# willow-ahrens/ChainPartitioners.jl

Measured on AMD Instinct MI355X. Metric: partitions/sec, DynamicTotalSplitter(AffineConnectivityModel{Int64}(0,0,0,1)), K=64, higher is better.
Workload: dtype int64; 1 GPU; config 3: DynamicTotalSplitter(AffineConnectivityModel{Int64}(0,0,0,1)) on suitesparse_shaped CSR (seeded SplitMix64 generator, tests/synth.py), n=10000000 rows, nnz=100000000, K=64; one independent partition per GPU; n=10000000, nnz=100000000, K=64, includes_oracle_build=True, device_block_pool=True

## Files before the change

### chainpartitioners.jl_amd/csrc/dp_total.hip

```cpp
#include "csr.hpp"
#include "model.hpp"
#include "dp.hpp"
#include <algorithm>

namespace cpk {

template <typename TC>
__device__ __forceinline__ TC dm_apply_affine(const DevModel<TC> &m, TC alpha, int64_t nv, int64_t np, int64_t nn, int64_t nl)
{
    TC v = cadd(cadd(alpha, cmulc(nv, m.p[CP_P_VERTEX])), cmulc(np, m.p[CP_P_PIN]));
    if (m.kind == CP_MODEL_CONNECTIVITY) return cadd(v, cmulc(nn, m.p[CP_P_NET]));
    if (m.kind == CP_MODEL_HYPEREDGE_CUT) return cadd(cadd(v, cmulc(nl, m.p[CP_P_SELF_NET])), cmulc(nn - nl, m.p[CP_P_CUT_NET]));
    return v;
}
#define dm_apply dm_apply_affine

constexpr int LT = 256;
constexpr int NBMAX = 31;
constexpr int SPLIT_BMIN = 8;
constexpr int SPLIT_NB = NBMAX - SPLIT_BMIN;

__device__ __forceinline__ int64_t prow(int64_t r, int64_t n)
{
    int t = __ffsll((long long)r) - 1;
// ... 558 lines not shown
    }
}

__device__ __forceinline__ void load_tile_tasks(const int64_t *__restrict__ offs, int64_t ntask, int64_t t0, int64_t tile_start,
                                                bool active, int32_t *s_off, unsigned long long *s_hd, int lane, int &cnt)
{
    int64_t c = ntask - t0;
    cnt = active ? (int)(c > LT + 1 ? LT + 1 : c) : 0;
    if (lane < LT / 64) s_hd[lane] = 0ull;
    for (int i = lane; i < cnt; i += 64) {
        int64_t rel = offs[t0 + i] - tile_start;
        if (rel < -(int64_t)0x3fffffff) rel = -(int64_t)0x3fffffff;
        if (rel > (int64_t)0x3fffffff) rel = (int64_t)0x3fffffff;
        s_off[i] = (int32_t)rel;
        if (rel >= 0 && rel < LT) atomicOr(&s_hd[rel >> 6], 1ull << (rel & 63));
    }
}

template <bool GE>
__device__ __forceinline__ int32_t coop_count(const int32_t *__restrict__ arr, int32_t s, int32_t en, int32_t thr, bool valid, int lane)
{
    int32_t prev_s = __shfl_up(s, 1);
    int prev_valid = __shfl_up((int)valid, 1);
    bool cont = valid && lane > 0 && prev_valid && (en == prev_s);
    unsigned long long heads = __ballot(valid && !cont);
    unsigned long long vm = __ballot(valid);
    int32_t d = 0;
    const int32_t FILL = GE ? INT32_MIN : INT32_MAX;
    while (heads) {
        int h0 = __ffsll((long long)heads) - 1;
        heads &= heads - 1;
        int h1 = heads ? (__ffsll((long long)heads) - 1) : 64;
        unsigned long long inrun = vm & (h1 == 64 ? ~0ull : ((1ull << h1) - 1)) & ~((1ull << h0) - 1);
        int hl = 63 - __clzll((long long)inrun);
        int32_t q_hi = __shfl(en, h0), q_lo = __shfl(s, hl);
        bool mine = lane >= h0 && lane <= hl && en > s;
        for (int32_t x = q_lo & ~3; x < q_hi; x += 512) {
            int4 v0 = make_int4(FILL, FILL, FILL, FILL), v1 = v0;
            int32_t b0 = x + 4 * lane, b1 = b0 + 256;
            if (b0 < q_hi) v0 = *reinterpret_cast<const int4 *>(arr + b0);
            if (b1 < q_hi) v1 = *reinterpret_cast<const int4 *>(arr + b1);
#pragma unroll
            for (int c = 0; c < 2; c++) {
                int32_t xc = x + c * 256;
                if (xc >= q_hi) break;
                int4 v = c ? v1 : v0;
                bool ov = mine && s < xc + 256 && en > xc;
                int a0 = ov ? ((s > xc ? s : xc) - xc) : 0, a1 = ov ? ((en < xc + 256 ? en : xc + 256) - xc) : 0;
                unsigned long long rem = __ballot(ov);
                while (rem) {
                    int l = __ffsll((long long)rem) - 1;
                    int32_t tu = __shfl(thr, l);
                    const bool f0 = GE ? v.x >= tu : v.x < tu, f1 = GE ? v.y >= tu : v.y < tu, f2 = GE ? v.z >= tu : v.z < tu, f3 = GE ? v.w >= tu : v.w < tu;
                    const unsigned long long m0 = __ballot(f0), m1 = __ballot(f1), m2 = __ballot(f2), m3 = __ballot(f3);
                    uint32_t P0 = 0;
                    P0 = __builtin_amdgcn_mbcnt_hi((uint32_t)(m0 >> 32), __builtin_amdgcn_mbcnt_lo((uint32_t)m0, P0));
                    P0 = __builtin_amdgcn_mbcnt_hi((uint32_t)(m1 >> 32), __builtin_amdgcn_mbcnt_lo((uint32_t)m1, P0));
                    P0 = __builtin_amdgcn_mbcnt_hi((uint32_t)(m2 >> 32), __builtin_amdgcn_mbcnt_lo((uint32_t)m2, P0));
                    P0 = __builtin_amdgcn_mbcnt_hi((uint32_t)(m3 >> 32), __builtin_amdgcn_mbcnt_lo((uint32_t)m3, P0));
                    const int32_t pack = (int32_t)((P0 << 3) | (uint32_t)f0 | ((uint32_t)f1 << 1) | ((uint32_t)f2 << 2));
                    const int32_t tot = __popcll(m0) + __popcll(m1) + __popcll(m2) + __popcll(m3);
                    const int32_t g0 = __shfl(pack, (a0 >> 2) & 63), g1 = __shfl(pack, (a1 >> 2) & 63);
                    bool same = ov && thr == tu;
                    if (same) {
                        int32_t F0 = (g0 >> 3) + __popc((uint32_t)g0 & ((1u << (a0 & 3)) - 1u));
                        int32_t F1 = a1 >= 256 ? tot : (g1 >> 3) + __popc((uint32_t)g1 & ((1u << (a1 & 3)) - 1u));
                        d += F1 - F0;
                    }
                    rem &= ~__ballot(same);
                }
            }
        }
    }
    return d;
}

constexpr int SMAX = 31;
template <bool GE, bool DET = false>
__device__ __forceinline__ void interior_stream(const int32_t *__restrict__ arr, const int32_t *__restrict__ cpos, int32_t p_first, int32_t tl,
                                                int32_t thr, int lane, int32_t acc[4], int32_t sk[4], int head = 0, int32_t sp_lo = 0, int32_t sp_hi = 0,
                                                int32_t *s_es = nullptr, int32_t *s_v = nullptr, int32_t *s_cnt = nullptr, int kind = 0,
                                                const int32_t *__restrict__ psum = nullptr)
{
    const int32_t FILL = GE ? INT32_MIN : INT32_MAX;
    const int32_t ptop = psum ? psum[p_first + 1 - head] : 0;
#pragma unroll
    for (int k = 0; k < 4; k++) {
        int32_t e = lane + 64 * k;
        sk[k] = e <= tl ? cpos[p_first - e] : INT32_MAX;
        acc[k] = (psum && e <= tl) ? ptop - psum[p_first - e] : 0;
    }
    int32_t Q_hi = cpos[p_first + 1 - head], Q_lo = cpos[p_first - tl];
    int32_t x = Q_lo & ~3;
    int4 c0 = make_int4(FILL, FILL, FILL, FILL), c1 = c0;
    if (x + 4 * lane < Q_hi) c0 = *reinterpret_cast<const int4 *>(arr + x + 4 * lane);
    if (x + 256 + 4 * lane < Q_hi) c1 = *reinterpret_cast<const int4 *>(arr + x + 256 + 4 * lane);
    for (; x < Q_hi; x += 512) {
        int4 n0 = make_int4(FILL, FILL, FILL, FILL), n1 = n0;
        if (x + 512 + 4 * lane < Q_hi) n0 = *reinterpret_cast<const int4 *>(arr + x + 512 + 4 * lane);
        if (x + 768 + 4 * lane < Q_hi) n1 = *reinterpret_cast<const int4 *>(arr + x + 768 + 4 * lane);
#pragma unroll
        for (int c = 0; c < 2; c++) {
            int32_t xc = x + c * 256;
            if (xc >= Q_hi) break;
            int4 v = c ? c1 : c0;
            int32_t pb = xc + 4 * lane;
            const bool inner = xc >= Q_lo && xc + 256 <= Q_hi;
            bool f0 = GE ? v.x >= thr : v.x < thr, f1 = GE ? v.y >= thr : v.y < thr, f2 = GE ? v.z >= thr : v.z < thr, f3 = GE ? v.w >= thr : v.w < thr;
            if (!inner) { f0 = f0 && pb < Q_hi; f1 = f1 && pb + 1 < Q_hi; f2 = f2 && pb + 2 < Q_hi; f3 = f3 && pb + 3 < Q_hi; }
            const unsigned long long m0 = __ballot(f0), m1 = __ballot(f1), m2 = __ballot(f2), m3 = __ballot(f3);
            if (DET) {
                const uint32_t span = (uint32_t)(sp_hi - sp_lo - 1);
                bool s0 = (uint32_t)(v.x - sp_lo - 1) < span, s1 = (uint32_t)(v.y - sp_lo - 1) < span, s2 = (uint32_t)(v.z - sp_lo - 1) < span,
                     s3 = (uint32_t)(v.w - sp_lo - 1) < span;
                if (!inner) {
                    s0 = s0 && pb >= Q_lo && pb < Q_hi; s1 = s1 && pb + 1 >= Q_lo && pb + 1 < Q_hi;
                    s2 = s2 && pb + 2 >= Q_lo && pb + 2 < Q_hi; s3 = s3 && pb + 3 >= Q_lo && pb + 3 < Q_hi;
                }
                if (s0 || s1 || s2 || s3) {
#pragma unroll
                    for (int j = 0; j < 4; j++) {
                        if (j == 0 ? s0 : j == 1 ? s1 : j == 2 ? s2 : s3) {
                            int32_t val = j == 0 ? v.x : j == 1 ? v.y : j == 2 ? v.z : v.w;
                            int slot = atomicAdd(s_cnt, 1);
                            if (slot <= SMAX - 1) {
                                s_es[slot] = pb + j;
                                s_v[slot] = (int32_t)(((uint32_t)val & 0x7fffffffu) | ((uint32_t)kind << 31));
                            }
                        }
                    }
                }
            }
            int32_t tot = __popcll(m0) + __popcll(m1) + __popcll(m2) + __popcll(m3);
            uint32_t P0 = 0;
            P0 = __builtin_amdgcn_mbcnt_hi((uint32_t)(m0 >> 32), __builtin_amdgcn_mbcnt_lo((uint32_t)m0, P0));
            P0 = __builtin_amdgcn_mbcnt_hi((uint32_t)(m1 >> 32), __builtin_amdgcn_mbcnt_lo((uint32_t)m1, P0));
            P0 = __builtin_amdgcn_mbcnt_hi((uint32_t)(m2 >> 32), __builtin_amdgcn_mbcnt_lo((uint32_t)m2, P0));
            P0 = __builtin_amdgcn_mbcnt_hi((uint32_t)(m3 >> 32), __builtin_amdgcn_mbcnt_lo((uint32_t)m3, P0));
            const int32_t pack = (int32_t)((P0 << 3) | (uint32_t)f0 | ((uint32_t)f1 << 1) | ((uint32_t)f2 << 2));
#pragma unroll
            for (int k = 0; k < 4; k++) {
                int32_t idx = sk[k] - xc;
                bool inside = idx > 0 && idx < 256;
                if (__ballot(inside)) {
                    int32_t cidx = inside ? idx : 0;
                    int src = cidx >> 2, comp = cidx & 3;
                    const int32_t g = __shfl(pack, src);
                    int32_t Fb = (g >> 3) + __popc((uint32_t)g & ((1u << comp) - 1u));
                    acc[k] += idx <= 0 ? tot : (inside ? tot - Fb : 0);
                } else {
                    acc[k] += idx <= 0 ? tot : 0;
                }
            }
        }
        c0 = n0; c1 = n1;
    }
}

constexpr int FIX_SERIAL = 16;
constexpr int FIX_U = 8;
constexpr int FIX_TRIP = 256 * FIX_U;
__global__ void __launch_bounds__(256) k_own_map(RoundCounts *__restrict__ rc, const int64_t *__restrict__ toffs, const int4 *__restrict__ tdesc,
                                                 const int32_t *__restrict__ rlen, int4 *__restrict__ rec, int32_t *__restrict__ tile_task,
                                                 const uint8_t *__restrict__ tb, int32_t *__restrict__ gap_hi, int tau, int64_t n, int blk,
                                                 int32_t *__restrict__ bcnt, int32_t *__restrict__ brank, int2 *__restrict__ items,
                                                 int32_t *__restrict__ item_of, int split)
{
    const int64_t ntask = rc->nown, ntile = rc->NT;
    for (int64_t tile = (int64_t)blockIdx.x * blockDim.x + threadIdx.x; tile < ntile; tile += (int64_t)gridDim.x * blockDim.x) {
    int64_t lo = 0, hi = ntask;
    while (hi - lo > 1) {
        int64_t mid = (lo + hi) >> 1;
        if (toffs[mid] <= tile) lo = mid; else hi = mid;
    }
    int32_t kt = (int32_t)(tile - toffs[lo]);
    if (items) {
        const bool first = kt % FIX_TRIP == 0 && toffs[lo + 1] - toffs[lo] > FIX_SERIAL;
        const unsigned long long mf = __ballot(first);
        if (mf) {
            const int lane = threadIdx.x & 63, lead = __ffsll((long long)mf) - 1;
            int32_t base = 0;
            if (lane == lead) base = atomicAdd(&rc->n_items, (int32_t)__popcll(mf));
            base = __shfl(base, lead);
            if (first) {
                const int32_t it = base + __popcll(mf & ((1ull << lane) - 1ull));
                items[it] = make_int2((int32_t)lo, kt);
                item_of[tile] = it;
            }
        }
    }
    int4 td = tdesc[lo];
    int32_t pf, tl;
    own_tile_geo(blk, td.x, rlen[lo], kt, pf, tl);
    const bool isgap = gap_hi != nullptr;
    const int sb = (split && tb[lo] >= SPLIT_BMIN) ? tb[lo] : 0;
    rec[tile] = make_int4(pf, td.z, td.w, (sb << 10) | (tl << 2) | (isgap ? 2 : 0) | (kt == 0 ? 1 : 0));
    if (split == 2) {
        const unsigned long long ms = __ballot(sb != 0);
        if (ms && (int)(threadIdx.x & 63) == __ffsll((long long)ms) - 1) atomicAdd(&rc->n_split, (int32_t)__popcll(ms));
    }
    tile_task[tile] = (int32_t)lo;
    if (bcnt) brank[tile] = atomicAdd(&bcnt[pf / LT], 1);
    if (isgap) {
        int64_t r = td.z, b = tb[lo];
        int64_t hi = r + ((int64_t)1 << tau), re = (((r >> b) + 1) << b);
        if (hi > re) hi = re;
        if (hi > n + 1) hi = n + 1;
        gap_hi[tile] = (int32_t)hi;
    }
    }
}

__global__ void __launch_bounds__(256) k_blk_order(const RoundCounts *__restrict__ rc, const int4 *__restrict__ rec, const int32_t *__restrict__ brank,
                                                   const int64_t *__restrict__ bstart, int32_t *__restrict__ border, int32_t *__restrict__ bcnt)
{
    const int64_t ntile = rc->NT;
    for (int64_t tile = (int64_t)blockIdx.x * blockDim.x + threadIdx.x; tile < ntile; tile += (int64_t)gridDim.x * blockDim.x) {
        const int32_t c = rec[tile].x / LT, rk = brank[tile];
        border[bstart[c] + rk] = (int32_t)tile;
        if (rk == 0) bcnt[c] = 0;
    }
}

template <typename TC, bool HYP, bool GAP>
__global__ void __launch_bounds__(256) k_lpass_own(int isA, const RoundCounts *__restrict__ rc, const int32_t *__restrict__ border,
                                                   const int32_t *__restrict__ a_pos, const int32_t *__restrict__ a_next,
                                                   const int32_t *__restrict__ a_fpos, const int32_t *__restrict__ a_flast,
                                                   int32_t *__restrict__ a_tileS, int32_t *__restrict__ a_tileS2, const int4 *__restrict__ a_rec,
                                                   const TC *__restrict__ W, DevModel<TC> M, TC alpha, Best<TC, HYP> *__restrict__ part,
                                                   int tau, const int32_t *__restrict__ gap_hi, uint8_t *__restrict__ spec, int force_spec,
                                                   Best<TC, HYP> *__restrict__ sub, int32_t *__restrict__ spv,
                                                   const int32_t *__restrict__ a_col, const int32_t *__restrict__ a_ffirst,
                                                   const int32_t *__restrict__ a_vnext, const int32_t *__restrict__ a_vpos,
                                                   const int32_t *__restrict__ a_vsa, int64_t vstride)
{
    int lane = threadIdx.x & 63;
    int64_t tile = (int64_t)blockIdx.x * 4 + (threadIdx.x >> 6);
    if (tile >= rc->NT) return;
    if (border) tile = border[tile];
    int4 rec = a_rec[tile];
    const int32_t rw = __builtin_amdgcn_readfirstlane(rec.w);
    int head = rw & 1;
    int32_t tl = (rw >> 2) & 255;
    int32_t acc[4], acc2[4] = {0, 0, 0, 0}, sk[4], sk2[4];
    __shared__ int32_t s_es_all[4][2][SMAX + 1], s_v_all[4][2][SMAX + 1];
    __shared__ int32_t s_cnt_all[4];
    int32_t(*s_es)[SMAX + 1] = s_es_all[threadIdx.x >> 6], (*s_v)[SMAX + 1] = s_v_all[threadIdx.x >> 6];
    int ns = 0;
    if (GAP && (rw & 2)) {
        int32_t *s_cnt = &s_cnt_all[threadIdx.x >> 6];
        if (lane == 0) *s_cnt = 0;
        __threadfence_block();
        int32_t rL = rec.y - (1 << tau), hi1 = gap_hi[tile] - 1;
        interior_stream<true, true>(a_next, a_pos, rec.x, tl, hi1, lane, acc, sk, head, rL, hi1, s_es[0], s_v[0], s_cnt, 0);
        if (HYP) interior_stream<false, true>(a_flast, a_fpos, rec.x, tl, rL + 1, lane, acc2, sk2, head, rL, hi1, s_es[0], s_v[0], s_cnt, 1);
        __threadfence_block();
        ns = *s_cnt;
        if (force_spec) ns = SMAX + 1;
        if (ns > 0 && ns <= SMAX) {
            if (lane < ns) {
                const int32_t q = s_es[0][lane];
                const bool k1 = s_v[0][lane] < 0;
                s_es[0][lane] = rec.x - (k1 ? a_ffirst[q] : a_col[q]);
            }
            __threadfence_block();
        }
    } else if (!HYP && !GAP) {
        const int sb = rw >> 10;
        const int64_t so = sb ? (int64_t)(sb - SPLIT_BMIN) * vstride : 0;
        interior_stream<true>(sb ? a_vnext : a_next, sb ? a_vpos + so : a_pos, rec.x, tl, rec.y, lane, acc, sk, head, 0, 0, nullptr, nullptr, nullptr, 0,
                              sb ? a_vsa + so : (const int32_t *)nullptr);
        if (sb) {
#pragma unroll
            for (int k = 0; k < 4; k++) if (lane + 64 * k <= tl) sk[k] = a_pos[rec.x - lane - 64 * k];
        }
    } else {
        interior_stream<true>(a_next, a_pos, rec.x, tl, rec.y, lane, acc, sk, head);
        if (HYP) interior_stream<false>(a_flast, a_fpos, rec.x, tl, rec.y, lane, acc2, sk2, head);
    }
    int sel = tl >> 6;
    if (lane == (tl & 63)) {
        a_tileS[tile] = sel == 0 ? acc[0] : sel == 1 ? acc[1] : sel == 2 ? acc[2] : acc[3];
        if (HYP) a_tileS2[tile] = sel == 0 ? acc2[0] : sel == 1 ? acc2[1] : sel == 2 ? acc2[2] : acc2[3];
    }
    Best<TC, HYP> cand[4];
#pragma unroll
    for (int k = 0; k < 4; k++) {
        int32_t e = lane + 64 * k;
        best_clear(cand[k]);
        if (e <= tl && !(head && isA && e == 0)) {
            int32_t p = rec.x - e;
            TC fv = dm_apply(M, alpha, (int64_t)(rec.y - p), (int64_t)(rec.z - sk[k]), (int64_t)acc[k], (int64_t)acc2[k]);
            cand[k].v = cadd(W[p], fv); cand[k].p = p; cand[k].nn = acc[k]; best_set_nl(cand[k], acc2[k]);
        }
    }
    if (GAP && ns > SMAX) {
        if (lane == 0) spec[tile] = 255;
        return;
    }
    if (!GAP || ns == 0) {
        Best<TC, HYP> best; best_clear(best);
#pragma unroll
        for (int k = 0; k < 4; k++) best = better(best, cand[k]);
        for (int o = 32; o > 0; o >>= 1) {
            int src = (lane + o) & 63;
            Best<TC, HYP> c; best_clear(c); c.v = shfl64(best.v, src); c.p = __shfl(best.p, src); c.nn = __shfl(best.nn, src);
            if (HYP) best_set_nl(c, __shfl(best_nl(best), src));
            bool take = (best.p < 0) ? (c.p >= 0) : (c.p >= 0 && (c.v < best.v || (c.v == best.v && c.p > best.p)));
            if (lane + o < 64 && take) best = c;
        }
        if (lane == 0) { part[tile] = best; if (GAP) spec[tile] = 0; }
        return;
    }
    __threadfence_block();
    if (lane < ns) {
        int32_t es_i = s_es[0][lane]; int rank = 0;
        for (int j = 0; j < ns; j++) { int32_t es_j = s_es[0][j]; rank += (es_j < es_i) || (es_j == es_i && j < lane); }
        s_es[1][rank] = es_i; s_v[1][rank] = s_v[0][lane];
    }
    __threadfence_block();
    int seg[4] = {0, 0, 0, 0}, hd[5] = {0, 0, 0, 0, 0};
    for (int i = 0; i < ns; i++) {
        int32_t es_i = s_es[1][i];
#pragma unroll
        for (int k = 0; k < 4; k++) { seg[k] += (es_i <= lane + 64 * k); hd[k] |= (es_i == lane + 64 * k); }
    }
    if (lane == 0) hd[0] = 1;
    const int64_t sbase = tile * (SMAX + 1);
    if (lane <= ns) {
        int32_t lo = lane == 0 ? 0 : s_es[1][lane - 1], hi = lane == ns ? tl + 1 : s_es[1][lane];
        if (hi <= lo) { Best<TC, HYP> z; best_clear(z); sub[sbase + lane] = z; }
    }
    Best<TC, HYP> bcarry; best_clear(bcarry);
#pragma unroll
    for (int k = 0; k < 4; k++) {
        int32_t e = lane + 64 * k;
        Best<TC, HYP> x = cand[k];
        int f = hd[k];
        wave_segmin<TC, HYP>(x, f, lane);
        if (!f) x = better(bcarry, x);
        {
            Best<TC, HYP> nb; best_clear(nb); nb.v = shfl64(x.v, 63); nb.p = __shfl(x.p, 63); nb.nn = __shfl(x.nn, 63);
            if (HYP) best_set_nl(nb, __shfl(best_nl(x), 63));
            bcarry = nb;
        }
        int nh = __shfl_down(hd[k], 1), nh0 = __shfl(hd[k + 1], 0);
        if (lane == 63) nh = nh0;
        if (e <= tl && (e == tl || nh)) sub[sbase + seg[k]] = x;
    }
    if (lane < ns) spv[sbase + lane] = s_v[1][lane];
    if (lane == 0) spec[tile] = (uint8_t)ns;
}

template <bool GE>
__device__ __forceinline__ int32_t gap_right_counts(const int32_t *__restrict__ cpos, const int32_t *__restrict__ arr, int32_t rL, int ck, int32_t thr,
                                                    int32_t n, int lane)
{
    int32_t cfirst = rL + 64 * ck;
    if (cfirst > n) cfirst = n;
    int32_t c = 0;
    for (int32_t q = cpos[rL] + lane, q1 = cpos[cfirst]; q < q1; q += 64) { int32_t v = arr[q]; c += GE ? (v >= thr) : (v < thr); }
    for (int o = 32; o > 0; o >>= 1) c += __shfl_xor(c, o);
    int32_t jn = cfirst + lane + 1, cl = cfirst + 64;
    if (jn > n) jn = n;
    if (cl > n) cl = n;
    const int32_t myend = cpos[jn], e0 = cpos[cfirst], e1 = cpos[cl];
    int32_t mine = 0;
    for (int32_t base = e0; base < e1; base += 256) {
        bool fl[4];
#pragma unroll
        for (int j = 0; j < 4; j++) {
            int32_t q = base + 64 * j + lane;
            fl[j] = false;
            if (q < e1) { int32_t v = arr[q]; fl[j] = GE ? (v >= thr) : (v < thr); }
        }
#pragma unroll
// ... 1455 lines not shown
            if (dst >= 0) vnext[dst] = x;
        }
}

static void split_build(cp_csr_s *A, SplitLinks &S, DBuf<int64_t> &scratch)
{
    hipStream_t s = A->stream;
    const int64_t n = A->n, n1 = n + 1;
    int nbits = 1;
    while (((int64_t)1 << nbits) <= n) nbits++;
    S.nb = std::max(0, nbits - SPLIT_BMIN); S.stride = n1;
    for (auto &t : S.tot) t = 0;
    if (S.nb > 0) {
        CP_REQUIRE(S.nb <= SPLIT_NB, CP_EINVAL, "n exceeds the bit-plane budget");
        const size_t cells = (size_t)S.nb * (size_t)n1;
        S.vpos.ensure(cells + 1); S.vsa.ensure(cells + 1); S.vnext.ensure((size_t)A->N + 8);
        const unsigned grid = (unsigned)cdiv(n1, 256);
        hipLaunchKernelGGL(k_split_count, dim3(grid), dim3(256), 0, s, A->pos32.p, A->next.p, n, S.nb, S.vsa.p);
        exclusive_scan_i32_i32(S.vsa.p, S.vpos.p, (int64_t)cells, scratch, s);
        hipLaunchKernelGGL(k_split_scatter, dim3(grid), dim3(256), 0, s, A->pos32.p, A->next.p, n, S.nb, S.vpos.p, S.vnext.p, S.vsa.p);
        CP_HIP(hipGetLastError());
        int32_t st[SPLIT_NB + 1];
        for (int b = 0; b <= S.nb; b++)
            CP_HIP(hipMemcpyAsync(&st[b], S.vpos.p + (size_t)b * (size_t)n1, sizeof(int32_t), hipMemcpyDeviceToHost, s));
        CP_HIP(hipStreamSynchronize(s));
        for (int b = 0; b < S.nb; b++) S.tot[b] = (int64_t)st[b + 1] - st[b];
        S.tot[S.nb] = st[S.nb];
    }
    S.built = true;
}

void dp_own_split_test(cp_csr_s *A, int32_t *vpos_out, int32_t *vsa_out, int32_t *vnext_out, int64_t *res)
{
    ensure_links(A);
    SplitLinks S;
    DBuf<int64_t> scratch;
    split_build(A, S, scratch);
    res[0] = S.nb; res[1] = S.tot[S.nb];
    if (S.nb <= 0) return;
    const size_t cells = (size_t)S.nb * (size_t)S.stride;
    CP_HIP(hipMemcpyAsync(vpos_out, S.vpos.p, cells * sizeof(int32_t), hipMemcpyDeviceToHost, A->stream));
    CP_HIP(hipMemcpyAsync(vsa_out, S.vsa.p, cells * sizeof(int32_t), hipMemcpyDeviceToHost, A->stream));
    if (res[1] > 0) CP_HIP(hipMemcpyAsync(vnext_out, S.vnext.p, (size_t)res[1] * sizeof(int32_t), hipMemcpyDeviceToHost, A->stream));
    CP_HIP(hipStreamSynchronize(A->stream));
}

template <typename TC>
struct LayerWork {
    int64_t n = -1; int nbits = 0; bool hyp = false;
    DBuf<int32_t> opt, nnopt, cr, len, loc, tileS;
    DBuf<int4> tdesc;
    DBuf<int32_t> nlopt, crl, tS0l, loc2, tileS2;
    DBuf<uint8_t> tb;
    DBuf<int64_t> offs, scratch, taskR, tilePS, tilePS2, tile_t0;
    ScanWS scanws;
    DBuf<Best<TC, true>> partL, partR;
    DBuf<int32_t> open_list, fix_list;
    DBuf<int4> tile_rec;
    DBuf<int4> o_tdesc, o_rec;
    DBuf<uint8_t> o_tb;
    DBuf<int32_t> o_rlen, o_ntl, o_tS0l, o_task, o_tileS, o_tileS2, o_hi;
    DBuf<int2> o_items; DBuf<int32_t> o_item_of; DBuf<unsigned long long> o_trec; DBuf<uint32_t> o_tick;
    bool t_dirty = true;
    DBuf<Best<TC, true>> o_sub;
    DBuf<int32_t> o_spv;
    bool ra_built = false; RATab ra_tab; int64_t ra_ntile = 0, ra_nrow = 0;
    SplitLinks split;
    bool mir_built = false; RATab mir_tab; int64_t mir_ntile = 0, mir_nrow = 0, mir_w = 0;
    DBuf<int32_t> mir_c, mir_c2;
    DBuf<Best<TC, true>> mir_part;
    DBuf<int32_t> ra_c, ra_c2;
    DBuf<int64_t> ra_G;
    DBuf<Best<TC, true>> ra_part;
    DBuf<int2> g_slot;
    DBuf<int2> g_list;
    DBuf<char> g_seg;
    DBuf<int32_t> g_slow, g_sslow;
    DBuf<int32_t> last_s0;
    DBuf<uint8_t> o_spec, fin;
    int fin_stamp = 255;
    DBuf<int64_t> o_toffs, o_tilePS, o_tilePS2;
    DBuf<Best<TC, true>> o_part;
    DBuf<int32_t> b_cnt, b_n, o_brank, o_border;
    DBuf<int64_t> b_start;
    int64_t b_nblk = 0;
    bool b_dirty = true;
    int64_t max_tasks = 0;
    bool planes_full = false;
    DBuf<int32_t> pz;
    Geo G{0, 0, 0};
    bool win_built = false; int64_t win_w = -1, win_nitems = 0, win_aoff[33];
    DBuf<int32_t> w_anch, w_anch2, w_tot, w_hist;
    DBuf<int32_t> leaf_anch, leaf_anch2;
    DBuf<int64_t> w_E;
    DBuf<RoundCounts> rc;
    std::vector<RoundCounts> pred;
    bool pred_ok = false; int64_t pred_rlo = 0, pred_rhi = 0; double pred_scale = 1.0; int pred_win = 0; int64_t pred_w = 0;
    std::vector<uint8_t> force_own;
    int64_t force_rows = 0;
    void forget() { ra_built = false; split.built = false; pred_ok = false; win_built = false; mir_built = false; force_own.clear(); force_rows = 0; }
    void ensure_own(size_t NT) {
        if (o_rec.n >= NT && o_rec.n > 0) return;
        size_t c = NT > 0 ? NT : 1;
        o_rec.release();
        o_task.alloc(c); o_tileS.alloc(c); o_tilePS.alloc(c + 1); o_part.alloc(c); o_hi.alloc(c); o_spec.alloc(c); o_brank.alloc(c); o_border.alloc(c);
        o_item_of.alloc(c); o_items.alloc(fix_items_cap(c)); o_trec.alloc(fix_items_cap(c) * FIX_REC_W);
        o_sub.alloc(c * (SMAX + 1)); o_spv.alloc(c * (SMAX + 1));
        if (hyp) { o_tileS2.alloc(c); o_tilePS2.alloc(c + 1); }
        o_rec.alloc(c);
    }
    void ensure_flat(size_t T) {
        if (loc.n >= T && loc.n > 0) return;
        size_t c = T > 0 ? T : 1, nt = (c + LT - 1) / LT;
        loc.release();
        if (hyp) loc2.alloc(c);
        tileS.alloc(nt); tilePS.alloc(nt + 1); tile_t0.alloc(nt); partL.alloc(nt); partR.alloc(nt); taskR.alloc(nt);
        open_list.alloc(nt); fix_list.alloc(nt); tile_rec.alloc(nt);
        if (hyp) { tileS2.alloc(nt); tilePS2.alloc(nt + 1); }
        loc.alloc(c);
    }
};

template <bool HYP, typename TC> static Best<TC, HYP> *recs(const DBuf<Best<TC, true>> &b) { return reinterpret_cast<Best<TC, HYP> *>(b.p); }
template <bool HYP, typename T> static T *if_hyp(T *p) { return HYP ? p : nullptr; }

static int64_t count_rows(int b, int tau, int64_t x)
{
    if (x < 0) return 0;
    int sh = b - tau - 1;
    int64_t V = (int64_t)1 << sh;
    int64_t nfull = (x + ((int64_t)1 << tau)) >> (b + 1);
    int64_t cnt = nfull * V;
    int64_t y = x - (nfull << (b + 1)) - ((int64_t)1 << b);
    if (y >= ((int64_t)1 << tau)) cnt += ((y >> tau) + 1) >> 1;
    return cnt;
}

static void make_round(RoundDesc &R, bool isA, int tau, int nbits, int64_t n, int64_t rlo, int64_t rhi, const Geo &G = Geo{0, 0, 0},
                       const int64_t *aoff = nullptr)
{
    memset(&R, 0, sizeof(R));
    R.isA = isA; R.tau = tau; R.nbits = nbits; R.n = n; R.G = G;
    if (G.win) {
        if (aoff) for (int b = 0; b < 32; b++) R.aoff[b] = aoff[b];
        int64_t acc = 0;
        for (int b = 0; b < 36; b++) {
            R.tbase[b] = acc;
            if (b > G.s || (!isA && b <= tau)) continue;
            if (isA) {
                int64_t lo = rlo - ((int64_t)2 << b), hi = rhi + ((int64_t)1 << b);
                if (lo < ((int64_t)1 << b)) lo = (int64_t)1 << b;
                if (hi > n) hi = n;
                int64_t l0 = ((lo + ((int64_t)1 << b) - 1) >> b) - 1, l1 = (hi >> b) - 1;
                R.tskip[b] = l0;
                acc += l1 >= l0 ? l1 - l0 + 1 : 0;
            } else {
                int64_t rmin = rlo - ((int64_t)1 << tau), rmax = rhi + ((int64_t)1 << tau);
                if (rmax > n) rmax = n;
                int64_t u0 = rmin <= 0 ? 0 : (((rmin - 1) >> tau) + 1) >> 1, u1 = ((rmax >> tau) + 1) >> 1;
                R.tskip[b] = u0;
                acc += u1 > u0 ? u1 - u0 : 0;
            }
        }
        R.ntask = acc;
        return;
    }
    if (isA) {
        int64_t r0 = rlo > 1 ? rlo : 1, r1 = rhi < n ? rhi : n;
        R.a_r0 = r0; R.a_nmain = r1 >= r0 ? r1 - r0 + 1 : 0;
        R.nextra = 0;
        for (int b = 0; b < nbits; b++) {
            int64_t step = (int64_t)1 << b;
            for (int side = 0; side < 2; side++) {
                int64_t lo = side == 0 ? rlo - step : rhi + 1, hi = side == 0 ? rlo - 1 : rhi + step;
                if (lo < 1) lo = 1;
                if (hi > n) hi = n;
                for (int64_t r = ((lo + step - 1) >> b) << b; r <= hi; r += step)
                    if (r >= 1 && ((r >> b) & 1) && R.nextra < 64) R.extra[R.nextra++] = r;
            }
        }
        R.nlast = 0;
        if (n >= 1) {
            int lowest = 0;
            while (!((n >> lowest) & 1)) lowest++;
            for (int b = lowest + 1; b < nbits; b++) if ((n >> b) & 1) R.last_b[R.nlast++] = b;
        }
        R.ntask = R.a_nmain + R.nextra + R.nlast;
        return;
// ... 301 lines not shown
                        elems += (double)std::max<int64_t>(0, T3.thi[b] - T3.tlo[b]) * LT;
                    }
                    const bool mcols = !(g_opt_dbg & DBG_MIR_ROWMAJOR);
                    const int64_t zt0 = r_lo / LT, zt1 = cdiv(std::min<int64_t>(n + G.w + 1, r_hi + ((int64_t)1 << G.s) + 1), LT);
                    ProfScope ps2(PROF_RA, s, mcols ? 80.0 * (double)(zt1 - zt0) * LT : 16.0 * elems);
                    launch_round_a<TC, HYP>(s, A, Wk, W, M, alpha, T3, Wk.mir_c, Wk.mir_c2, Wk.mir_part, Wk.mir_ntile, Wk.mir_nrow, zt0, zt1, 0, true, mcols);
                    R.skip_mir = 1;
                }
            }
        }
        if (R.ntask <= 0) continue;
        CP_REQUIRE(R.ntask <= Wk.max_tasks, CP_EINTERNAL, "a DP round has more tasks than the task buffers hold");
        RoundCounts *rc = Wk.rc.p + rd;
        const bool gap = gaps && !R.isA && R.tau <= g_opt_gap_tau;
        const bool forced = allow_force && own_tiles && !gap && !R.isA && (size_t)rd < Wk.force_own.size() && Wk.force_own[(size_t)rd] &&
                            (rhi - rlo + 1) <= 2 * Wk.force_rows && !(g_opt_dbg & DBG_NO_FORCE_OWN);
        any_forced |= forced;
        if (!R.isA) {
            int64_t cols = (((n >> R.tau) + 1) >> 1) << R.tau;
            ProfScope ps(PROF_RPASS, s, 4.0 * (avg_deg + self_deg) * (double)cols + 8.0 * (double)R.ntask);
            if (((int64_t)1 << R.tau) > g_opt_rpass_ch)
                hipLaunchKernelGGL(k_setup, dim3((unsigned)cdiv(R.ntask, 256)), dim3(256), 0, s, R, Wk.opt.p, Wk.nnopt.p, Wk.cr.p, 1,
                                   Wk.tdesc.p, A->pos32.p, Wk.tb.p, Wk.len.p, (const int32_t *)nullptr, if_hyp<HYP>(Wk.crl.p), (int32_t *)nullptr);
            launch_rpass(s, R, nbits, n, rlo, rhi, A->pos.p, A->prev.p, 0, Wk.opt.p, Wk.cr.p, avg_deg);
            if (hyp) launch_rpass(s, R, nbits, n, rlo, rhi, A->lpos.p, A->lfirst.p, 1, Wk.opt.p, Wk.crl.p, self_deg);
        }
        if (R.isA && R.nlast > 0) {
            CP_HIP(hipMemsetAsync(Wk.last_s0.p, 0, Wk.last_s0.bytes(), s));
            hipLaunchKernelGGL(k_last_row_counts, dim3(1024), dim3(256), 0, s, R, A->pos32.p, A->prev.p, if_hyp<HYP>(A->lpos32.p), if_hyp<HYP>(A->lfirst.p),
                               Wk.last_s0.p, Wk.fin.p);
        }
        {
            ProfScope ps(PROF_SETUP, s, 29.0 * (double)R.ntask);
            const int sbs = (int)g_opt_setup_bs;
            dim3 sgrid((unsigned)cdiv(R.ntask, sbs));
            if (!R.isA) {
                int64_t mx = 1;
                for (int bb = R.tau + 1; bb < nbits; bb++) mx = std::max<int64_t>(mx, R.tbase[bb + 1] - R.tbase[bb]);
                sgrid = dim3((unsigned)cdiv(mx, sbs), (unsigned)std::max(1, nbits - R.tau - 1));
            }
            hipLaunchKernelGGL(HIP_KERNEL_NAME(k_setup_short<TC, HYP>), sgrid, dim3(sbs), 0, s, R, Wk.opt.p, Wk.nnopt.p, Wk.nlopt.p, Wk.cr.p, Wk.crl.p, A->pos32.p,
                               A->next.p, if_hyp<HYP>(A->fpos32.p), if_hyp<HYP>(A->flast.p), W, M, alpha, Wk.tdesc.p, Wk.tb.p, Wk.len.p, Wk.tS0l.p, &rc->nlong,
                               (int32_t)g_opt_short_t, (int32_t)g_opt_short_e, own_tiles ? Wk.o_tdesc.p : (int4 *)nullptr, Wk.o_tb.p, Wk.o_rlen.p, Wk.o_ntl.p,
                               Wk.o_tS0l.p, &rc->nown, &rc->own_steps, (int32_t)(forced ? 2 : gap ? g_opt_gap_min : g_opt_own_min),
                               (int32_t)std::min<size_t>(Wk.o_ntl.n, (size_t)INT32_MAX), &rc->err, Wk.fin.p, Wk.last_s0.p,
                               (g_opt_dbg & DBG_COUNT_NONTRIVIAL) ? &rc->_pad : (int32_t *)nullptr, Wk.w_anch.p, Wk.w_anch2.p, pzp, oblk);
        }
        RoundCounts P;
        if (spec) {
            P = Wk.pred[(size_t)rd];
            if (Wk.pred_scale != 1.0) {
                auto sc = [&](int64_t v) { return (int64_t)((double)v * Wk.pred_scale) + (v > 0 ? 1 : 0); };
                P.nlong = (int32_t)sc(P.nlong); P.nown = (int32_t)sc(P.nown); P.T = sc(P.T); P.NT = sc(P.NT);
                P.own_steps = (unsigned long long)sc((int64_t)P.own_steps);
            }
            if ((g_opt_dbg & DBG_MISPREDICT) && (rd & 1)) { P.nown = 0; P.NT = 0; P.nlong = 0; P.T = 0; }
            Wk.ensure_own((size_t)grow(P.NT));
            Wk.ensure_flat((size_t)grow(P.T));
        }
        {
            ProfScope ps(PROF_SCAN, s, 12.0 * (double)R.ntask);
            const bool tiny = spec && (g_opt_dbg & DBG_TINY_BUFFERS);
            const int64_t capT = spec ? (tiny ? (int64_t)64 : (int64_t)Wk.loc.n) : INT64_MAX, capNT = spec ? (tiny ? (int64_t)1 : (int64_t)Wk.o_rec.n) : INT64_MAX;
            const int64_t nm = std::min<int64_t>(R.ntask, (int64_t)Wk.o_ntl.n);
            if (R.ntask <= LB_MAX) {
                launch_round_scans(rc, Wk.len.p, Wk.offs.p, R.ntask, Wk.o_ntl.p, Wk.o_toffs.p, nm, own_tiles, capT, capNT, Wk.scanws, s);
            } else {
                exclusive_scan_i32_devn(Wk.len.p, Wk.offs.p, &rc->nlong, R.ntask, &rc->T, Wk.scratch, s);
                if (own_tiles) exclusive_scan_i32_devn(Wk.o_ntl.p, Wk.o_toffs.p, &rc->nown, nm, &rc->NT, Wk.scratch, s);
                hipLaunchKernelGGL(k_round_finish, dim3(1), dim3(1), 0, s, rc, capT, capNT);
            }
        }
        if (!spec) {
            CP_HIP(hipMemcpyAsync(&P, rc, sizeof(P), hipMemcpyDeviceToHost, s));
            CP_HIP(hipStreamSynchronize(s));
            Wk.ensure_own((size_t)P.NT);
            Wk.ensure_flat((size_t)P.T);
        }
        used[(size_t)rd] = P;
        if (g_opt_dbg & DBG_PRINT_ROUNDS) fprintf(stderr, "round isA=%d tau=%d ntask=%lld %s long=%d own=%d T=%lld NT=%lld nontrivial=%d\n", R.isA, R.tau, (long long)R.ntask,
                                   spec ? "predicted" : "exact", P.nlong, P.nown, (long long)P.T, (long long)P.NT, P._pad);
        if (P.nown > 0 && P.NT > 0) {
            const int64_t gNT = spec ? (int64_t)Wk.o_rec.n : P.NT, gown = spec ? grow(P.nown) : P.nown;
            poison_fill(s, {{Wk.o_part.p, Wk.o_part.bytes()}, {Wk.o_tileS.p, Wk.o_tileS.bytes()}, {Wk.o_rec.p, Wk.o_rec.bytes()},
                            {if_hyp<HYP>(Wk.o_tileS2.p), Wk.o_tileS2.bytes()}, {Wk.o_items.p, Wk.o_items.bytes()}, {Wk.o_item_of.p, Wk.o_item_of.bytes()},
                            {Wk.o_trec.p, Wk.o_trec.bytes()}});
            const unsigned mgrid = (unsigned)std::min<int64_t>(cdiv(gNT, 256), 8192);
            const int split = !(split_layer && !gap && !R.isA) ? 0 : R.tau + 1 >= SPLIT_BMIN ? 1 : 2;
            split_mode[(size_t)rd] = (int8_t)split;
            if (split && !Wk.split.built) {
                ProfScope ps(PROF_LINKS, s, 8.0 * (double)A->N + 16.0 * (double)(nbits - SPLIT_BMIN) * (double)(n + 1));
                split_build(A, Wk.split, Wk.scratch);
            }
            hipLaunchKernelGGL(k_own_map, dim3(mgrid), dim3(256), 0, s, rc, Wk.o_toffs.p, Wk.o_tdesc.p, Wk.o_rlen.p, Wk.o_rec.p, Wk.o_task.p,
                               Wk.o_tb.p, gap ? Wk.o_hi.p : (int32_t *)nullptr, R.tau, n, oblk, oblk ? Wk.b_cnt.p : (int32_t *)nullptr, Wk.o_brank.p,
                               gap ? (int2 *)nullptr : Wk.o_items.p, Wk.o_item_of.p, split);
            {
                ProfScope ps(gap ? PROF_GAPSTREAM : PROF_OWN, s, own_bytes(R.tau, split != 0, (double)P.own_steps));
                if (oblk) {
                    exclusive_scan_i32_lb(Wk.b_cnt.p, Wk.b_start.p, Wk.b_n.p, Wk.b_nblk, nullptr, Wk.scanws, s);
                    hipLaunchKernelGGL(k_blk_order, dim3(mgrid), dim3(256), 0, s, rc, Wk.o_rec.p, Wk.o_brank.p, Wk.b_start.p, Wk.o_border.p, Wk.b_cnt.p);
                }
                hipLaunchKernelGGL(HIP_KERNEL_NAME(gap ? k_lpass_own<TC, HYP, true> : k_lpass_own<TC, HYP, false>), dim3((unsigned)cdiv(gNT, 4)), dim3(256), 0, s,
                                   R.isA, rc,
                                   oblk ? Wk.o_border.p : (const int32_t *)nullptr, A->pos32.p, A->next.p, if_hyp<HYP>(A->fpos32.p), if_hyp<HYP>(A->flast.p),
                                   Wk.o_tileS.p, Wk.o_tileS2.p, Wk.o_rec.p, W, M, alpha, recs<HYP>(Wk.o_part), R.tau, Wk.o_hi.p, Wk.o_spec.p,
                                   (int)((g_opt_dbg & DBG_GAP_ALL_SPECIAL) != 0), recs<HYP>(Wk.o_sub), Wk.o_spv.p, A->col.p, if_hyp<HYP>(A->ffirst.p),
                                   split ? Wk.split.vnext.p : (const int32_t *)nullptr, Wk.split.vpos.p, Wk.split.vsa.p, (int64_t)(n + 1));
            }
            note(rd, 0, gap ? PROF_GAPSTREAM : PROF_OWN, R.tau, split != 0);
            if (gap) {
                {
                    ProfScope ps(PROF_CARRY, s, 12.0 * (double)P.NT);
                    const int32_t *ntp = reinterpret_cast<const int32_t *>(&rc->NT);
                    exclusive_scan_i32_lb(Wk.o_tileS.p, Wk.o_tilePS.p, ntp, (int64_t)Wk.o_tileS.n, nullptr, Wk.scanws, s);
                    if (hyp) exclusive_scan_i32_lb(Wk.o_tileS2.p, Wk.o_tilePS2.p, ntp, (int64_t)Wk.o_tileS.n, nullptr, Wk.scanws, s);
                }
                ProfScope ps(PROF_GAP, s, 24.0 * (double)P.NT);
                const int nchunk = (int)std::max<int64_t>(1, ((int64_t)2 << R.tau) / 64);
                const size_t ncap = Wk.o_rec.n / GAPSEG + 2;
                Wk.g_list.ensure(ncap); Wk.g_slot.ensure(2 * ncap);
                Wk.g_seg.ensure((2 * ncap) * (size_t)nchunk * 64 * sizeof(GapSegRec<TC, true>));
                Wk.g_slow.ensure((size_t)gown * (size_t)nchunk + 64); Wk.g_sslow.ensure((2 * ncap) * (size_t)nchunk + 64);
                CP_REQUIRE((int64_t)gown * nchunk < INT32_MAX && (int64_t)(2 * ncap) * nchunk < INT32_MAX, CP_EINTERNAL, "gap work index beyond 32 bits");
                const int gnr = (g_opt_gap_nr >= 2 && nchunk >= 2) ? 2 : 1;
                unsigned gg = (unsigned)std::min<int64_t>(cdiv(gown * cdiv((int64_t)nchunk, gnr), 4), 16384);
                unsigned gs_grid = (unsigned)std::min<int64_t>(cdiv((int64_t)(2 * ncap) * nchunk, 4), 8192);
                unsigned gm = (unsigned)std::min<int64_t>(cdiv((int64_t)ncap * nchunk, 4), 4096);
                const unsigned gslow_grid = 2048;
                launch_gap<TC, HYP>(s, A, Wk, R.tau, nchunk, gnr, rc, n, W, M, alpha, gg, gs_grid, gm, gslow_grid, oblk);
            } else {
                ProfScope ps(PROF_FIX, s, 24.0 * (double)P.NT);
                launch_fix_own<TC, HYP>(s, rc, Wk.o_toffs.p, recs<HYP>(Wk.o_part), Wk.o_tdesc.p, Wk.o_tb.p, if_hyp<HYP>(Wk.o_tS0l.p), Wk.o_tileS.p,
                                        if_hyp<HYP>(Wk.o_tileS2.p), M, Wk.opt.p, Wk.nnopt.p, if_hyp<HYP>(Wk.nlopt.p), n, Wk.o_items.p, Wk.o_item_of.p, Wk.o_trec.p,
                                        Wk.o_tick.p, spec ? grow(P.NT) : P.NT, gown);
            }
            CP_HIP(hipGetLastError());
        }
        if (P.nlong <= 0 || P.T <= 0) continue;
        const int64_t gtile = spec ? (int64_t)Wk.tileS.n : cdiv(P.T, LT);
        poison_fill(s, {{Wk.loc.p, Wk.loc.bytes()}, {if_hyp<HYP>(Wk.loc2.p), Wk.loc2.bytes()}, {Wk.partL.p, Wk.partL.bytes()}, {Wk.partR.p, Wk.partR.bytes()},
                        {Wk.tileS.p, Wk.tileS.bytes()}, {if_hyp<HYP>(Wk.tileS2.p), Wk.tileS2.bytes()}});
        hipLaunchKernelGGL(k_tile_t0, dim3((unsigned)cdiv(gtile, 256)), dim3(256), 0, s, rc, Wk.offs.p, Wk.tdesc.p, Wk.tile_t0.p,
                           Wk.tile_rec.p, (int)((g_opt_dbg & DBG_NO_INTERIOR) != 0), Wk.taskR.p);
        {
            ProfScope ps(PROF_EXPAND, s, (double)P.T * step_bytes);
            hipLaunchKernelGGL(HIP_KERNEL_NAME(k_lpass<TC, HYP>), dim3((unsigned)cdiv(gtile, 4)), dim3(256), 0, s, R, rc, Wk.offs.p, Wk.tdesc.p, Wk.tS0l.p, Wk.tb.p,
                               A->pos32.p, A->next.p, if_hyp<HYP>(A->fpos32.p), if_hyp<HYP>(A->flast.p), Wk.opt.p, Wk.nnopt.p, Wk.nlopt.p, Wk.loc.p, Wk.loc2.p,
                               Wk.tileS.p, Wk.tileS2.p, Wk.taskR.p, Wk.tile_t0.p, Wk.tile_rec.p, W, M, alpha, recs<HYP>(Wk.partR), recs<HYP>(Wk.partL));
        }
        note(rd, 1, PROF_EXPAND);
        {
            ProfScope ps(PROF_CARRY, s, 12.0 * (double)cdiv(P.T, LT));
            exclusive_scan_i32_lb(Wk.tileS.p, Wk.tilePS.p, &rc->ntile, (int64_t)Wk.tileS.n, nullptr, Wk.scanws, s);
            if (hyp) exclusive_scan_i32_lb(Wk.tileS2.p, Wk.tilePS2.p, &rc->ntile, (int64_t)Wk.tileS.n, nullptr, Wk.scanws, s);
        }
        unsigned wgrid = (unsigned)std::min<int64_t>(cdiv(gtile, 4), 8192);
        {
            ProfScope ps(PROF_EVAL, s, 0.0);
            hipLaunchKernelGGL(HIP_KERNEL_NAME(k_span_short<TC, HYP>), dim3((unsigned)cdiv(gtile, 256)), dim3(256), 0, s, R, rc, Wk.offs.p, Wk.tdesc.p, Wk.tS0l.p,
                               Wk.tb.p, A->pos32.p, Wk.loc.p, Wk.loc2.p, Wk.tile_t0.p, Wk.taskR.p, Wk.tileS.p, Wk.tileS2.p, recs<HYP>(Wk.partR), W, M, alpha,
                               Wk.opt.p, Wk.nnopt.p, if_hyp<HYP>(Wk.nlopt.p), Wk.open_list.p, Wk.fix_list.p, Wk.tile_rec.p);
            hipLaunchKernelGGL(HIP_KERNEL_NAME(k_open<TC, HYP>), dim3(wgrid), dim3(256), 0, s, R, rc, Wk.offs.p, Wk.tdesc.p, Wk.tS0l.p, A->pos32.p, Wk.loc.p,
                               Wk.loc2.p, Wk.tile_t0.p, Wk.tilePS.p, if_hyp<HYP>(Wk.tilePS2.p), W, M, alpha, recs<HYP>(Wk.partL), Wk.open_list.p);
        }
        {
            ProfScope ps(PROF_FIX, s, 8.0 * (double)cdiv(P.T, LT));
            hipLaunchKernelGGL(HIP_KERNEL_NAME(k_fix<TC, HYP>), dim3(wgrid), dim3(256), 0, s, rc, Wk.offs.p, Wk.taskR.p, recs<HYP>(Wk.partL), recs<HYP>(Wk.partR),
                               Wk.tdesc.p, Wk.tb.p, Wk.opt.p, Wk.nnopt.p, if_hyp<HYP>(Wk.nlopt.p), n + 1, Wk.fix_list.p, Wk.tile_rec.p, Wk.tilePS.p,
                               if_hyp<HYP>(Wk.tilePS2.p), if_hyp<HYP>(Wk.tS0l.p), M);
        }
        CP_HIP(hipGetLastError());
    }
    if (leaf) {
        const int64_t c0 = rlo > 1 ? rlo : 1, c1 = rhi < n ? rhi : n;
        if (c1 >= c0) {
            const int64_t g0 = c0 >> LEAF_T, g1 = c1 >> LEAF_T;
            ProfScope ps(PROF_LEAF, s, (8.0 * (avg_deg + self_deg) + 4.0 + 8.0 + 12.0) * (double)((g1 - g0 + 1) << LEAF_T));
            const int need = G.win ? G.s - LEAF_T + 2 : nbits - LEAF_T;
            CP_REQUIRE(need <= 25, CP_EINTERNAL, "leaf pass: more outer planes than counters");
            const int32_t lcap = (gaps && g_opt_gap_tau >= LEAF_T) ? (int32_t)std::max<int64_t>(g_opt_gap_min, 2) : INT32_MAX;
            LeafArgs<TC, HYP> L{};
            L.n = n; L.g0 = g0; L.ngroups = g1 - g0 + 1; L.c0 = c0; L.c1 = c1; L.nbits = nbits; L.planes = (int32_t)(g_opt_block_tables != 0);
            L.pos = A->pos32.p; L.prev = A->prev.p; L.next = A->next.p; L.col = A->col.p;
            L.fpos = if_hyp<HYP>(A->fpos32.p); L.flast = if_hyp<HYP>(A->flast.p); L.ffirst = if_hyp<HYP>(A->ffirst.p);
            L.lpos = if_hyp<HYP>(A->lpos32.p); L.lfirst = if_hyp<HYP>(A->lfirst.p);
            L.opt = Wk.opt.p; L.nnopt = Wk.nnopt.p; L.nlopt = if_hyp<HYP>(Wk.nlopt.p); L.fin = Wk.fin.p; L.fin_stamp = Wk.fin_stamp;
            L.W = W; L.M = M; L.alpha = alpha; L.cst = cst_out; L.ptr = ptr_out; L.G = G;
            L.anchM = Wk.leaf_anch.p; L.anchM2 = if_hyp<HYP>(Wk.leaf_anch2.p); L.lcap = lcap; L.err = &Wk.rc.p->err; L.pz = pzp;
// ... 176 lines not shown
```

Baseline: 2.335 partitions/s.

## Make streaming loads branch-free and store tile records in block order

The interior stream loader now clamps its load offsets instead of predicating them. It hoists wave-uniform values into scalar registers with readfirstlane and issues all cpos/psum loads before using them. The block-ordering kernel also writes a copy of each tile record into a block-sorted array, so the own-pass kernel reads its record directly instead of through the indirection. The W values and split-path sk values are prefetched with clamped, branchless loads. Clamped loads read some duplicate or extra elements beyond the valid range, which relies on the masking downstream. The extra srec array adds memory traffic in k_blk_order.

```diff
diff --git a/chainpartitioners.jl_amd/csrc/dp_total.hip b/chainpartitioners.jl_amd/csrc/dp_total.hip
--- a/chainpartitioners.jl_amd/csrc/dp_total.hip
+++ b/chainpartitioners.jl_amd/csrc/dp_total.hip
@@ -664,23 +664,31 @@
                                                 int32_t *s_es = nullptr, int32_t *s_v = nullptr, int32_t *s_cnt = nullptr, int kind = 0,
                                                 const int32_t *__restrict__ psum = nullptr)
 {
-    const int32_t FILL = GE ? INT32_MIN : INT32_MAX;
-    const int32_t ptop = psum ? psum[p_first + 1 - head] : 0;
+    p_first = __builtin_amdgcn_readfirstlane(p_first);
+    tl = __builtin_amdgcn_readfirstlane(tl) & 255;
+    const int32_t *__restrict__ cl = cpos + (p_first - tl), *__restrict__ pl = (psum ? psum : cpos) + (p_first - tl);
+    int32_t cp[4], pv[4];
 #pragma unroll
     for (int k = 0; k < 4; k++) {
-        int32_t e = lane + 64 * k;
-        sk[k] = e <= tl ? cpos[p_first - e] : INT32_MAX;
-        acc[k] = (psum && e <= tl) ? ptop - psum[p_first - e] : 0;
-    }
-    int32_t Q_hi = cpos[p_first + 1 - head], Q_lo = cpos[p_first - tl];
+        const int32_t e = lane + 64 * k;
+        const uint32_t d = (uint32_t)(tl - (e < tl ? e : tl)) & 255u;
+        cp[k] = cl[d];
+        pv[k] = pl[d];
+    }
+    const int32_t ptop = pl[tl + 1 - head];
+    const int32_t Q_hi = __builtin_amdgcn_readfirstlane(cl[tl + 1 - head]), Q_lo = __builtin_amdgcn_readfirstlane(cl[0]);
+#pragma unroll
+    for (int k = 0; k < 4; k++) {
+        const bool on = lane + 64 * k <= tl;
+        sk[k] = on ? cp[k] : INT32_MAX;
+        acc[k] = (psum && on) ? ptop - pv[k] : 0;
+    }
+    const int32_t x_end = Q_hi & ~3;
     int32_t x = Q_lo & ~3;
-    int4 c0 = make_int4(FILL, FILL, FILL, FILL), c1 = c0;
-    if (x + 4 * lane < Q_hi) c0 = *reinterpret_cast<const int4 *>(arr + x + 4 * lane);
-    if (x + 256 + 4 * lane < Q_hi) c1 = *reinterpret_cast<const int4 *>(arr + x + 256 + 4 * lane);
+    auto quad = [&](uint32_t o) { const uint32_t r = (uint32_t)(x_end - x); return *reinterpret_cast<const int4 *>(arr + x + (o < r ? o : r)); };
+    int4 c0 = quad(4 * lane), c1 = quad(256 + 4 * lane);
     for (; x < Q_hi; x += 512) {
-        int4 n0 = make_int4(FILL, FILL, FILL, FILL), n1 = n0;
-        if (x + 512 + 4 * lane < Q_hi) n0 = *reinterpret_cast<const int4 *>(arr + x + 512 + 4 * lane);
-        if (x + 768 + 4 * lane < Q_hi) n1 = *reinterpret_cast<const int4 *>(arr + x + 768 + 4 * lane);
+        const int4 n0 = quad(512 + 4 * lane), n1 = quad(768 + 4 * lane);
 #pragma unroll
         for (int c = 0; c < 2; c++) {
             int32_t xc = x + c * 256;
@@ -794,12 +802,16 @@
 }
 
 __global__ void __launch_bounds__(256) k_blk_order(const RoundCounts *__restrict__ rc, const int4 *__restrict__ rec, const int32_t *__restrict__ brank,
-                                                   const int64_t *__restrict__ bstart, int32_t *__restrict__ border, int32_t *__restrict__ bcnt)
+                                                   const int64_t *__restrict__ bstart, int32_t *__restrict__ border, int4 *__restrict__ srec,
+                                                   int32_t *__restrict__ bcnt)
 {
     const int64_t ntile = rc->NT;
     for (int64_t tile = (int64_t)blockIdx.x * blockDim.x + threadIdx.x; tile < ntile; tile += (int64_t)gridDim.x * blockDim.x) {
-        const int32_t c = rec[tile].x / LT, rk = brank[tile];
-        border[bstart[c] + rk] = (int32_t)tile;
+        const int4 r = rec[tile];
+        const int32_t c = r.x / LT, rk = brank[tile];
+        const int64_t slot = bstart[c] + rk;
+        border[slot] = (int32_t)tile;
+        srec[slot] = r;
         if (rk == 0) bcnt[c] = 0;
     }
 }
@@ -809,7 +821,7 @@
                                                    const int32_t *__restrict__ a_pos, const int32_t *__restrict__ a_next,
                                                    const int32_t *__restrict__ a_fpos, const int32_t *__restrict__ a_flast,
                                                    int32_t *__restrict__ a_tileS, int32_t *__restrict__ a_tileS2, const int4 *__restrict__ a_rec,
-                                                   const TC *__restrict__ W, DevModel<TC> M, TC alpha, Best<TC, HYP> *__restrict__ part,
+                                                   const int4 *__restrict__ a_srec, const TC *__restrict__ W, DevModel<TC> M, TC alpha, Best<TC, HYP> *__restrict__ part,
                                                    int tau, const int32_t *__restrict__ gap_hi, uint8_t *__restrict__ spec, int force_spec,
                                                    Best<TC, HYP> *__restrict__ sub, int32_t *__restrict__ spv,
                                                    const int32_t *__restrict__ a_col, const int32_t *__restrict__ a_ffirst,
@@ -817,11 +829,12 @@
                                                    const int32_t *__restrict__ a_vsa, int64_t vstride)
 {
     int lane = threadIdx.x & 63;
-    int64_t tile = (int64_t)blockIdx.x * 4 + (threadIdx.x >> 6);
+    int64_t tile = (int64_t)blockIdx.x * 4 + __builtin_amdgcn_readfirstlane(threadIdx.x >> 6);
     if (tile >= rc->NT) return;
+    const int4 vrec = border ? a_srec[tile] : a_rec[tile];
     if (border) tile = border[tile];
-    int4 rec = a_rec[tile];
-    const int32_t rw = __builtin_amdgcn_readfirstlane(rec.w);
+    const int32_t rw = __builtin_amdgcn_readfirstlane(vrec.w);
+    const int4 rec = make_int4(__builtin_amdgcn_readfirstlane(vrec.x), __builtin_amdgcn_readfirstlane(vrec.y), __builtin_amdgcn_readfirstlane(vrec.z), rw);
     int head = rw & 1;
     int32_t tl = (rw >> 2) & 255;
     int32_t acc[4], acc2[4] = {0, 0, 0, 0}, sk[4], sk2[4];
@@ -852,14 +865,15 @@
         const int64_t so = sb ? (int64_t)(sb - SPLIT_BMIN) * vstride : 0;
         interior_stream<true>(sb ? a_vnext : a_next, sb ? a_vpos + so : a_pos, rec.x, tl, rec.y, lane, acc, sk, head, 0, 0, nullptr, nullptr, nullptr, 0,
                               sb ? a_vsa + so : (const int32_t *)nullptr);
-        if (sb) {
-#pragma unroll
-            for (int k = 0; k < 4; k++) if (lane + 64 * k <= tl) sk[k] = a_pos[rec.x - lane - 64 * k];
-        }
+#pragma unroll
+        for (int k = 0; k < 4; k++) { const int32_t e = lane + 64 * k; sk[k] = (a_pos + (rec.x - tl))[(uint32_t)(tl - (e < tl ? e : tl)) & 255u]; }
     } else {
         interior_stream<true>(a_next, a_pos, rec.x, tl, rec.y, lane, acc, sk, head);
         if (HYP) interior_stream<false>(a_flast, a_fpos, rec.x, tl, rec.y, lane, acc2, sk2, head);
     }
+    TC wv[4];
+#pragma unroll
+    for (int k = 0; k < 4; k++) { const int32_t e = lane + 64 * k; wv[k] = (W + (rec.x - tl))[(uint32_t)(tl - (e < tl ? e : tl)) & 255u]; }
     int sel = tl >> 6;
     if (lane == (tl & 63)) {
         a_tileS[tile] = sel == 0 ? acc[0] : sel == 1 ? acc[1] : sel == 2 ? acc[2] : acc[3];
@@ -873,7 +887,7 @@
         if (e <= tl && !(head && isA && e == 0)) {
             int32_t p = rec.x - e;
             TC fv = dm_apply(M, alpha, (int64_t)(rec.y - p), (int64_t)(rec.z - sk[k]), (int64_t)acc[k], (int64_t)acc2[k]);
-            cand[k].v = cadd(W[p], fv); cand[k].p = p; cand[k].nn = acc[k]; best_set_nl(cand[k], acc2[k]);
+            cand[k].v = cadd(wv[k], fv); cand[k].p = p; cand[k].nn = acc[k]; best_set_nl(cand[k], acc2[k]);
         }
     }
     if (GAP && ns > SMAX) {
@@ -2495,6 +2509,7 @@
     DBuf<int64_t> o_toffs, o_tilePS, o_tilePS2;
     DBuf<Best<TC, true>> o_part;
     DBuf<int32_t> b_cnt, b_n, o_brank, o_border;
+    DBuf<int4> o_srec;
     DBuf<int64_t> b_start;
     int64_t b_nblk = 0;
     bool b_dirty = true;
@@ -2516,7 +2531,7 @@
         if (o_rec.n >= NT && o_rec.n > 0) return;
         size_t c = NT > 0 ? NT : 1;
         o_rec.release();
-        o_task.alloc(c); o_tileS.alloc(c); o_tilePS.alloc(c + 1); o_part.alloc(c); o_hi.alloc(c); o_spec.alloc(c); o_brank.alloc(c); o_border.alloc(c);
+        o_task.alloc(c); o_tileS.alloc(c); o_tilePS.alloc(c + 1); o_part.alloc(c); o_hi.alloc(c); o_spec.alloc(c); o_brank.alloc(c); o_border.alloc(c); o_srec.alloc(c);
         o_item_of.alloc(c); o_items.alloc(fix_items_cap(c)); o_trec.alloc(fix_items_cap(c) * FIX_REC_W);
         o_sub.alloc(c * (SMAX + 1)); o_spv.alloc(c * (SMAX + 1));
         if (hyp) { o_tileS2.alloc(c); o_tilePS2.alloc(c + 1); }
@@ -2984,7 +2999,7 @@
                                    spec ? "predicted" : "exact", P.nlong, P.nown, (long long)P.T, (long long)P.NT, P._pad);
         if (P.nown > 0 && P.NT > 0) {
             const int64_t gNT = spec ? (int64_t)Wk.o_rec.n : P.NT, gown = spec ? grow(P.nown) : P.nown;
-            poison_fill(s, {{Wk.o_part.p, Wk.o_part.bytes()}, {Wk.o_tileS.p, Wk.o_tileS.bytes()}, {Wk.o_rec.p, Wk.o_rec.bytes()},
+            poison_fill(s, {{Wk.o_part.p, Wk.o_part.bytes()}, {Wk.o_tileS.p, Wk.o_tileS.bytes()}, {Wk.o_rec.p, Wk.o_rec.bytes()}, {Wk.o_srec.p, Wk.o_srec.bytes()},
                             {if_hyp<HYP>(Wk.o_tileS2.p), Wk.o_tileS2.bytes()}, {Wk.o_items.p, Wk.o_items.bytes()}, {Wk.o_item_of.p, Wk.o_item_of.bytes()},
                             {Wk.o_trec.p, Wk.o_trec.bytes()}});
             const unsigned mgrid = (unsigned)std::min<int64_t>(cdiv(gNT, 256), 8192);
@@ -3001,12 +3016,12 @@
                 ProfScope ps(gap ? PROF_GAPSTREAM : PROF_OWN, s, own_bytes(R.tau, split != 0, (double)P.own_steps));
                 if (oblk) {
                     exclusive_scan_i32_lb(Wk.b_cnt.p, Wk.b_start.p, Wk.b_n.p, Wk.b_nblk, nullptr, Wk.scanws, s);
-                    hipLaunchKernelGGL(k_blk_order, dim3(mgrid), dim3(256), 0, s, rc, Wk.o_rec.p, Wk.o_brank.p, Wk.b_start.p, Wk.o_border.p, Wk.b_cnt.p);
+                    hipLaunchKernelGGL(k_blk_order, dim3(mgrid), dim3(256), 0, s, rc, Wk.o_rec.p, Wk.o_brank.p, Wk.b_start.p, Wk.o_border.p, Wk.o_srec.p, Wk.b_cnt.p);
                 }
                 hipLaunchKernelGGL(HIP_KERNEL_NAME(gap ? k_lpass_own<TC, HYP, true> : k_lpass_own<TC, HYP, false>), dim3((unsigned)cdiv(gNT, 4)), dim3(256), 0, s,
                                    R.isA, rc,
                                    oblk ? Wk.o_border.p : (const int32_t *)nullptr, A->pos32.p, A->next.p, if_hyp<HYP>(A->fpos32.p), if_hyp<HYP>(A->flast.p),
-                                   Wk.o_tileS.p, Wk.o_tileS2.p, Wk.o_rec.p, W, M, alpha, recs<HYP>(Wk.o_part), R.tau, Wk.o_hi.p, Wk.o_spec.p,
+                                   Wk.o_tileS.p, Wk.o_tileS2.p, Wk.o_rec.p, Wk.o_srec.p, W, M, alpha, recs<HYP>(Wk.o_part), R.tau, Wk.o_hi.p, Wk.o_spec.p,
                                    (int)((g_opt_dbg & DBG_GAP_ALL_SPECIAL) != 0), recs<HYP>(Wk.o_sub), Wk.o_spv.p, A->col.p, if_hyp<HYP>(A->ffirst.p),
                                    split ? Wk.split.vnext.p : (const int32_t *)nullptr, Wk.split.vpos.p, Wk.split.vsa.p, (int64_t)(n + 1));
             }
```

Result: faster. 2.618 partitions/s (median of 6 runs) (+12.1%).
